# constantingoeldel/alphabeta-rs

Hardware: AMD Instinct MI355X
Metric: ABneutral model fits/sec (pedigree x bootstraps x windows) (higher is better)
Workload: dtype f64; 1 GPU; C3: synthetic 100-edge/8-generation pedigree (N=105 rows, T=8, K=47 distinct triples), 10 starts + 10000 bootstraps per GPU (bootstraps of one window sharded over the GPUs); rows=105, windows_per_gpu=1, starts=10, bootstraps=10000, plan_device_bytes=11405122, reduction_tree=0x10040, parallelism=bootstraps sharded over 1 GPU(s), one RCCL all-gather of the bootstrap tables

## Files before the change

### alphabeta_rs_amd/__init__.py

```python
from __future__ import annotations

import ctypes as C
import os
from pathlib import Path

import numpy as np

from . import build as _build

PKG = Path(__file__).resolve().parent
LIB_PATH = PKG / "libabneutral_hip.so"
if os.environ.get("ABNEUTRAL_HIP_LIB"):
    LIB_PATH = Path(os.environ["ABNEUTRAL_HIP_LIB"])

ABN_OK = 0
STATUS_NAMES = {
    0: "ABN_OK",
    1: "ABN_ERR_INVALID_ARG",
    2: "ABN_ERR_BAD_PEDIGREE",
    3: "ABN_ERR_NO_DEVICE",
    4: "ABN_ERR_HIP",
    5: "ABN_ERR_NO_FINITE_FIT",
    6: "ABN_ERR_STATE",
}
FIT_CONVERGED, FIT_MAX_ITERS, FIT_NONFINITE, FIT_TARGET = 0, 1, 2, 3
KERNEL_NAMES = {0: "none", 1: "speculative", 2: "resident", 3: "persistent", 4: "stream", 5: "two_pass",
                6: "stream_sweep"}

FIT_INFO_DTYPE = np.dtype(
    [("best_cost", "<f8"), ("iters", "<i4"), ("evals", "<i4"), ("status", "<i4"), ("lanes", "<i4")]
)

EXPORTED_SYMBOLS = [
    "abn_default_options", "abn_device_count", "abn_init", "abn_shutdown", "abn_device_info", "abn_last_error",
    "abn_status_string", "abn_version", "abn_cost_batch", "abn_fit_batch", "abn_gen_start_simplices",
    "abn_gen_boot_simplices", "abn_gen_boot_indices", "abn_ab_neutral_run", "abn_boot_model_run",
    "abn_analyze", "abn_select_best", "abn_bootstrap_rows", "abn_pairwise_divergence", "abn_plan_create", "abn_plan_destroy", "abn_plan_set_windows", "abn_plan_run",
    "abn_plan_run_phase", "abn_plan_sync", "abn_plan_tail_handed", "abn_plan_set_early_bootstraps", "abn_plan_early_bootstraps", "abn_plan_kernel_ms", "abn_plan_raw_device_ptr",
    "abn_plan_bind_raw", "abn_plan_download", "abn_plan_counters", "abn_plan_device_bytes",
    "abn_plan_set_window_ids", "abn_plan_failed_windows",
    "abn_multi_create", "abn_multi_destroy", "abn_multi_last_error", "abn_multi_set_windows", "abn_multi_run",
    "abn_multi_sync", "abn_multi_shard", "abn_multi_raw_device_ptr", "abn_multi_download", "abn_multi_counters",
    "abn_multi_rccl_available", "abn_reduction_tree", "abn_pairwise_divergence_dev", "abn_multi_set_window_ids",
    "abn_pairwise_divergence_windows", "abn_pairwise_divergence_windows_dev",
    "abn_multi_plan_shard", "abn_plan_last_kernels", "abn_multi_kernel_ms",
    "abn_packed_row_stride", "abn_pack_codes", "abn_unpack_codes", "abn_pairwise_divergence_packed",
    "abn_pairwise_divergence_packed_dev",
    "abn_pairwise_divergence_windows_packed", "abn_pairwise_divergence_windows_packed_dev",
    "abn_analyze_batch", "abn_analyze_batch_dev", "abn_plan_analyze", "abn_multi_analyze",
    "abn_windows_create", "abn_windows_destroy", "abn_windows_info", "abn_windows_stats", "abn_windows_layout",
    "abn_windows_packed", "abn_windows_packed_device_ptr", "abn_windows_pairwise",
    "abn_sites_parse", "abn_sites_destroy", "abn_sites_info", "abn_sites_fetch", "abn_sites_deferred",
    "abn_genes_create", "abn_genes_destroy", "abn_genes_choose", "abn_genes_choose_dev", "abn_windows_create_sites",
# ... 234 lines not shown
    L.abn_genes_create.argtypes = [vp, C.c_int32, i32p, i32p, i64p, u32p, u32p, u8p, C.POINTER(vp)]
    L.abn_genes_destroy.argtypes = [vp]
    L.abn_genes_choose.argtypes = [vp, C.POINTER(GeneRule), C.c_int32, i64p, i32p, u32p, u32p, u8p, u32p, u32p, u8p, dp]
    L.abn_genes_choose_dev.argtypes = [vp, C.POINTER(GeneRule), C.c_int32, i64p, vp, vp, vp, vp, vp, vp, vp, dp]
    L.abn_windows_create_sites.argtypes = [vp, C.POINTER(WindowsParams), vp, C.POINTER(GeneRule), C.c_int32, i64p, i32p,
                                           u32p, u32p, u8p, u8p, dp, C.POINTER(vp)]
    L.abn_plan_create.argtypes = [vp, op, dp, C.c_int32, C.c_int32, C.c_int32, C.c_int32, C.c_uint32, C.c_uint32,
                                  C.POINTER(vp)]
    L.abn_plan_destroy.argtypes = [vp]
    L.abn_plan_set_windows.argtypes = [vp, dp, dp, dp, dp]
    L.abn_plan_run.argtypes = [vp]
    L.abn_plan_run_phase.argtypes = [vp, C.c_int32]
    L.abn_plan_sync.argtypes = [vp]
    L.abn_plan_tail_handed.argtypes = [vp, C.POINTER(C.c_int64)]
    L.abn_plan_set_early_bootstraps.argtypes = [vp, C.c_int32]
    L.abn_plan_set_stream_sweep.argtypes = [vp, C.c_int32]
    L.abn_plan_stream_sweep.argtypes = [vp, C.POINTER(C.c_int64)]
    L.abn_multi_set_stream_sweep.argtypes = [vp, C.c_int32]
    L.abn_plan_early_bootstraps.argtypes = [vp, C.POINTER(C.c_int32)]
    L.abn_plan_kernel_ms.argtypes = [vp, dp]
    L.abn_plan_raw_device_ptr.argtypes = [vp, C.POINTER(vp)]
    L.abn_plan_bind_raw.argtypes = [vp, vp]
    L.abn_plan_download.argtypes = [vp, dp, dp, dp, dp, vp, vp, C.POINTER(C.c_int32)]
    L.abn_plan_counters.argtypes = [vp, C.POINTER(C.c_int64)]
    L.abn_plan_device_bytes.argtypes = [vp, C.POINTER(C.c_int64)]
    L.abn_plan_set_window_ids.argtypes = [vp, u32p]
    L.abn_plan_failed_windows.argtypes = [vp, C.POINTER(C.c_int32)]
    L.abn_plan_last_kernels.argtypes = [vp, C.POINTER(C.c_int32)]
    i32p = C.POINTER(C.c_int32)
    L.abn_multi_create.argtypes = [i32p, C.c_int32, op, dp, C.c_int32, C.c_int32, C.c_int32, C.c_int32, C.POINTER(vp)]
# ... 573 lines not shown

    def run_phase(self, phase: int):
        self.ctx._check(self._L.abn_plan_run_phase(self._h, phase))

    def sync(self):
        self.ctx._check(self._L.abn_plan_sync(self._h))

    def tail_handed(self):
        out = (C.c_int64 * 2)()
        self.ctx._check(self._L.abn_plan_tail_handed(self._h, out))
        return int(out[0]), int(out[1])

    def set_early_bootstraps(self, mode: int):
        self.ctx._check(self._L.abn_plan_set_early_bootstraps(self._h, mode))

    def early_bootstraps(self):
        out = (C.c_int32 * 4)()
        self.ctx._check(self._L.abn_plan_early_bootstraps(self._h, out))
        return {"eligible": bool(out[0]), "quorum": int(out[1]), "parked": int(out[2]), "miss": bool(out[3])}

    def set_stream_sweep(self, mode: int):
        self.ctx._check(self._L.abn_plan_set_stream_sweep(self._h, mode))

    def stream_sweep(self):
        out = (C.c_int64 * 4)()
        self.ctx._check(self._L.abn_plan_stream_sweep(self._h, out))
        return {"mode": int(out[0]), "starts": bool(out[1]), "boot": bool(out[2]), "passes": int(out[3])}

    def kernel_ms(self):
        ms = np.zeros(3)
# ... 684 lines not shown
```

### alphabeta_rs_amd/build.py

```python
from __future__ import annotations

import os
import shutil
import subprocess
from pathlib import Path

PKG = Path(__file__).resolve().parent
CSRC = PKG / "csrc"
LIB = PKG / "libabneutral_hip.so"
SOURCES = [CSRC / "abn_api.hip", CSRC / "abn_context.hip", CSRC / "abn_plan.hip",
           CSRC / "abn_pairwise.hip", CSRC / "abn_windows.hip", CSRC / "abn_analyze.hip",
           CSRC / "abn_multi.hip", CSRC / "abn_sites.hip", CSRC / "abn_genes.hip", CSRC / "abn_codes.hip",
           CSRC / "abn_sites_common.hip", CSRC / "abn_sites_union.hip", CSRC / "abn_tiles.hip", CSRC / "abn_blocks.hip",
           CSRC / "abn_sites_sort.hip",
           CSRC / "abn_resident.hip",
           CSRC / "abn_pack.cpp"]
DEPS = [*sorted(CSRC.glob("*.hpp")), CSRC / "abn_philox.h", PKG.parent / "include" / "abneutral.h"]
HIPCC_FLAGS = [
    "--offload-arch=gfx950",
    "-O3",
    "-std=c++17",
    "-ffp-contract=off",
    "-fno-fast-math",
    "-fPIC",
# ... 44 lines not shown
HOST = PKG / "host"
CLI = PKG / "bin" / "alphabeta"
META_CLI = PKG / "bin" / "metaprofile_alphabeta"
REF_TESTS = PKG / "bin" / "reference_tests"
PEDIGREE_LIB = PKG / "libabneutral_host.so"


def build_host(force: bool = False, verbose: bool = False) -> Path:
    build_hip()
    srcs = [HOST / "alphabeta_cli.cpp", HOST / "alphabeta.hpp", HOST / "pedigree_build.hpp", HOST / "windows_extract.hpp",
            HOST / "resident.hpp", HOST / "host_capi.cpp", HOST / "block_bootstrap.hpp",
            HOST / "metaprofile.hpp", HOST / "metaprofile_cli.cpp", HOST / "reference_tests.cpp",
            CSRC / "abn_route.hpp", CSRC / "abn_constants.hpp", CSRC / "abn_parse.hpp", CSRC / "abn_genes.hpp",
            CSRC / "abn_sites_merge.hpp", CSRC / "abn_sites_split.hpp", CSRC / "abn_sites_sort.hpp", CSRC / "abn_codes.hpp", CSRC / "abn_sites_common.hpp",
            CSRC / "abn_sites_union.hpp", CSRC / "abn_tiles.hpp", HOST / "tiles.hpp",
            CSRC / "abn_pairwise_transitions.hpp", CSRC / "abn_packed_mask.hpp", HOST / "transitions.hpp"]
    newest = max(p.stat().st_mtime for p in srcs)
    CLI.parent.mkdir(exist_ok=True)
    common = ["-O2", "-std=c++17", "-ffp-contract=off", "-Wall", "-I", str(PKG.parent / "include")]
    if force or not CLI.exists() or CLI.stat().st_mtime < newest:
        cmd = [hipcc_path(), *common, "-o", str(CLI), str(HOST / "alphabeta_cli.cpp"), "-L", str(PKG),
               "-labneutral_hip", "-Wl,-rpath,$ORIGIN/.."]
        if verbose:
            print(" ".join(cmd))
        subprocess.run(cmd, check=True, cwd=str(PKG))
    if force or not META_CLI.exists() or META_CLI.stat().st_mtime < newest:
        cmd = [hipcc_path(), *common, "-o", str(META_CLI), str(HOST / "metaprofile_cli.cpp"), "-L", str(PKG),
               "-labneutral_hip", "-Wl,-rpath,$ORIGIN/.."]
        if verbose:
            print(" ".join(cmd))
        subprocess.run(cmd, check=True, cwd=str(PKG))
# ... 19 lines not shown
```

### alphabeta_rs_amd/csrc/abn_api.hip

```cpp
#include <functional>

#include "abn_fit_host.hpp"
#include "abn_device.hpp"

using namespace abn;

static_assert(sizeof(abn_fit_info) == sizeof(FitInfoDev), "abn_fit_info layout");

static hipError_t allow_lds(const void* kernel, size_t lds) {
  if (lds <= kDefaultDynLds) return hipSuccess;
  return hipFuncSetAttribute(kernel, hipFuncAttributeMaxDynamicSharedMemorySize, (int)lds);
}

struct KernelEntry {
  KernelKey key;
  const void* fn;
};
#define ABN_FIT(G, R, TP, ST) {{kFamFit, G, R, TP, ST, false}, reinterpret_cast<const void*>(&abn_fit_kernel<G, R, TP, ST>)}
#define ABN_FIT_ROWS(G, TP, ST) ABN_FIT(G, 1, TP, ST), ABN_FIT(G, 2, TP, ST), ABN_FIT(G, 4, TP, ST), ABN_FIT(G, 8, TP, ST), ABN_FIT(G, 0, TP, ST)
#define ABN_FIT_G(G)                                                                                                   \
  ABN_FIT_ROWS(G, false, false), ABN_FIT(G, -1, false, false), ABN_FIT_ROWS(G, true, false), ABN_FIT(G, -1, true, false), \
      ABN_FIT_ROWS(G, false, true)
#define ABN_REFILL(G, R) {{kFamRefill, G, R, false, false, false}, reinterpret_cast<const void*>(&abn_fit_refill_kernel<G, R>)}
#define ABN_REFILL_G(G) ABN_REFILL(G, 1), ABN_REFILL(G, 2), ABN_REFILL(G, 4), ABN_REFILL(G, 8)
// ... 97 lines not shown
    const bool status = persistent && a.slice_status, fifo = a.quantum > 0;
    if ((status || fifo) && !lc) return set_err(c, ABN_ERR_INVALID_ARG, "internal: a persistent launch without its clears");
    if (lc) {
      bool& status_clean = lc->clean->status[lc->slot];
      bool& fifo_clean = lc->clean->fifo[lc->region];
      const PrepList l = prep_launch(lc->slot, status && !status_clean, fifo && !fifo_clean, (unsigned)a.park_cap, lc->region);
      if (int rc = clear_ranges(c, l, lc->bases, st)) return rc;
      if (status) status_clean = false;
      if (fifo) fifo_clean = false;
    }
  }
  if (int rc = launch_route(c, r, a, st)) return rc;
  if (a.tail_cap > 0) return launch_tail_resume(c, pr, a, a.tail_cap, st);
  return ABN_OK;
}

int abn::launch_select(abn_ctx* c, const SelectArgs& s, size_t lds, hipStream_t st) {
  HIPCHK(c, allow_lds(reinterpret_cast<const void*>(&abn_select_lse_kernel), lds));
  HIPCHK(c, allow_lds(reinterpret_cast<const void*>(&abn_select_kernel), lds));
  hipLaunchKernelGGL(abn_select_lse_kernel, dim3((unsigned)((long long)s.W * s.S)), dim3(kWave), lds, st, s);
  hipLaunchKernelGGL(abn_select_kernel, dim3((unsigned)s.W), dim3(kWave), lds, st, s);
  HIPCHK(c, hipGetLastError());
  return ABN_OK;
}

int abn::launch_gen_idx(abn_ctx* c, uint32_t* idx, int n, int b, int w, uint64_t seed, uint32_t woff, uint32_t boff,
                        const uint32_t* wid) {
  const long long total = (long long)w * b * ((n + 3) / 4);
  if (total <= 0) return ABN_OK;
  const long long want = (total + 255) / 256;
// ... 245 lines not shown
```

### alphabeta_rs_amd/csrc/abn_common.hpp

```cpp
#pragma once
#include <type_traits>
#include <hip/hip_runtime.h>
#include <stdint.h>

#include "abn_constants.hpp"
#include "abn_philox.h"

namespace abn {

#ifndef ABN_STREAM_WAVES
#define ABN_STREAM_WAVES 2
#endif
constexpr int kStreamWaves = ABN_STREAM_WAVES;

typedef uint32_t u32x4 __attribute__((ext_vector_type(4), aligned(4)));
typedef uint16_t u16x4 __attribute__((ext_vector_type(4), aligned(2)));
typedef double f64x2 __attribute__((ext_vector_type(2), aligned(8)));
typedef uint32_t u32x4_lds __attribute__((ext_vector_type(4)));
typedef double f64x2_lds __attribute__((ext_vector_type(2)));

constexpr int ST_INIT0 = 0;
constexpr int ST_REFLECT = 5;
constexpr int ST_EXPAND = 6;
constexpr int ST_CONTRACT = 7;
// ... 43 lines not shown
  int no_skip;
  unsigned long long* skipped;
  unsigned* queue;
  int quantum;
  unsigned park_cap;
  unsigned* park_ht;
  int* parked;
  unsigned* slice_status;
  int tail_cap;
  int spec_resume;
  unsigned* quorum_words;
  int quorum;
  const unsigned* guard;
  int guard_stop;
  int guard_poll;
#ifdef ABN_MEASUREMENT_KNOBS
  int prio_mode;
  int prio_t[3];
  int drop_entry;
#endif
  double sd_tol;
  double gap_tol;
  double* best;
  FitInfoDev* info;
  double* raw;
  unsigned long long* dbg;
  unsigned long long* passes;
};

struct SelectArgs {
// ... 264 lines not shown
__device__ __forceinline__ double cond_div(double a0, double a1, double a2, double b0, double b1, double b2) {
  return 0.5 * (a0 * b1 + a1 * b0 + a1 * b2 + a2 * b1) + (a0 * b2 + a2 * b0);
}

__device__ __forceinline__ void load_matrix(const double* m, double (&M)[9]) {
  const f64x2_lds* v = reinterpret_cast<const f64x2_lds*>(m);
#pragma unroll
  for (int e = 0; e < 4; ++e) {
    const f64x2_lds x = v[e];
    M[2 * e] = x[0];
    M[2 * e + 1] = x[1];
  }
  M[8] = m[8];
}

__device__ __forceinline__ double triple_dt(uint32_t tr, const double* pw, int TP, double sv0, double sv1,
                                            double sv2) {
  (void)TP;
  const int t0 = tr & 0xff, ea = (tr >> 8) & 0xff, eb = (tr >> 16) & 0xff;
  double P[9], A[9], B[9];
  load_matrix(pw + t0 * kPw, P);
  const double s0 = fma3(sv2, P[6], fma3(sv1, P[3], fma3(sv0, P[0], 0.0)));
  const double s1 = fma3(sv2, P[7], fma3(sv1, P[4], fma3(sv0, P[1], 0.0)));
  const double s2 = fma3(sv2, P[8], fma3(sv1, P[5], fma3(sv0, P[2], 0.0)));
  __builtin_amdgcn_sched_barrier(0);
  load_matrix(pw + ea * kPw, A);
  load_matrix(pw + eb * kPw, B);
  const double d_mm = cond_div(A[6], A[7], A[8], B[6], B[7], B[8]);
  const double d_um = cond_div(A[3], A[4], A[5], B[3], B[4], B[5]);
  const double d_uu = cond_div(A[0], A[1], A[2], B[0], B[1], B[2]);
  return s0 * d_uu + s1 * d_um + s2 * d_mm;
}

template <int I>
__device__ __forceinline__ void insert_tail(double (&c)[5], double (&v)[5]) {
  const double fi = c[I], xi = v[I];
  bool b[I];
  b[I - 1] = fi < c[I - 1];
#pragma unroll
  for (int j = I - 2; j >= 0; --j) b[j] = b[j + 1] && (fi < c[j]);
// ... 123 lines not shown
```

### alphabeta_rs_amd/csrc/abn_fit_refill.hpp

```cpp
#pragma once
#include "abn_common.hpp"
#include "abn_fit_kernel.hpp"

namespace abn {

constexpr int ST_IDLE = 13;

#ifndef ABN_REFILL_MIN_WAVES
#define ABN_REFILL_MIN_WAVES 3
#endif
typedef const __attribute__((address_space(4))) FitArgs ColdArgs;
template <int G, int RMAX>
__global__ __launch_bounds__(kWave, ABN_REFILL_MIN_WAVES) void abn_fit_refill_kernel(const FitArgs a) {
  static_assert(RMAX > 0, "resident mode only");
  constexpr int NG = kWave / G;
  constexpr int RR = RMAX;
  extern __shared__ __align__(16) double lds[];

  auto cold = [&]() {
    ColdArgs* p = (ColdArgs*)__builtin_amdgcn_kernarg_segment_ptr();
    asm volatile("" : "+s"(p));
    return p;
  };
  auto cold_v = [](int v) {
// ... 25 lines not shown
  double* dtab = pw + kPw * TP;
  double* wconst = dtab + ((K + 1) & ~1);
  double* dobs = wconst + 4;
  uint32_t* tri_s = reinterpret_cast<uint32_t*>(dobs + ((N + 1) & ~1));

  const bool canon = a.tree == kTreeCanon;
  uint32_t tidp[(RR + 1) / 2];
  for (int t = gl; t < K; t += G) tri_s[t] = a.tri[t];
#pragma unroll
  for (int q = 0; q < (RR + 1) / 2; ++q) tidp[q] = 0u;
#pragma unroll
  for (int q = 0; q < RR; ++q) {
    const int i = gl + G * q;
    if (i < N) tidp[q / 2] |= (uint32_t)a.tid[i] << (16 * (q & 1));
  }

  unsigned chain = blockIdx.x * NG + g;
  double vx[5], c[5];
  int st = ST_IDLE;
  int iter = 0, evals = 0;
  double xc = 0.0, x0 = 0.0, xr = 0.0, bx = __builtin_nan("");
  double fr = 0.0, best_cost = __builtin_inf();
  bool have_best = false;
  int fin_status = 2;
  int q_start = 0;
  bool fresh_done = false;
  bool wave_fd = false;
  bool tail_mode = false;
  bool tail_park = false;
  int skip_rest = 0;
  unsigned wstep = 0;
  unsigned gstep = 0;
#pragma unroll
  for (int k = 0; k < 5; ++k) {
    vx[k] = 0.0;
    c[k] = 0.0;
  }

  auto load_observations = [&](ColdArgs* ca, int w, int cgl) {
    const int wi = w * ca->wstride;
    const size_t wN = (size_t)w * (size_t)N;
    if (cgl == 0) {
      const double p_uu0 = ca->p_uu[wi];
      wconst[0] = p_uu0;
      wconst[1] = 1.0 - p_uu0;
      wconst[2] = ca->eqp[wi];
      wconst[3] = ca->eqp_w[wi] * (double)N;
    }
    const int dmode = ca->dmode;
    const uint32_t* idx_row = (dmode == 1) ? ca->idx + (size_t)chain * (size_t)N : nullptr;
    const size_t dN = (dmode == 2) ? (size_t)chain * (size_t)N : wN;
#pragma unroll
    for (int q = 0; q < RR; ++q) {
      const int i = cgl + G * q;
      if (i < N)
        dobs[i] = (dmode == 1) ? ca->pred[wN + i] + ca->resid[wN + idx_row[i]] : ca->D[dN + i];
    }
  };
  auto setup_chain = [&]() {
    ColdArgs* ca = cold();
    const int cgl = cold_v(gl), cdim = cgl & 3;
    const int w = (int)(chain / (unsigned)ca->C);
// ... 49 lines not shown
    fin_status = 2;
    fr = 0.0;
    double acc = vx[0];
    acc = acc + vx[1];
    acc = acc + vx[2];
    acc = acc + vx[3];
    x0 = acc * (1.0 / 4.0);
    xr = x0 + (x0 - vx[4]) * 1.0;
    xc = xr;
    q_start = evals;
    st = ST_REFLECT;
  };
  if (chain < total_of(cold())) setup_chain();
  __syncthreads();

  auto eval = [&](double xd) -> double {
    const double al = dpp_mov<kDppQuadBcast0>(xd), be = dpp_mov<kDppQuadBcast1>(xd);
    const double wt = dpp_mov<kDppQuadBcast2>(xd), ic = dpp_mov<kDppQuadBcast3>(xd);
    const double p_mm = wconst[1];
    const double sv0 = wconst[0], sv1 = wt * p_mm, sv2 = (1.0 - wt) * p_mm;
    const double puu = p_uu_est(al, be);
    const double dq = puu - wconst[2];
    const double pen = wconst[3] * (dq * dq);
    uint32_t tr = tri_s[gl < K ? gl : 0];
    const int T = (int)cold_s((unsigned)a.T);
    if constexpr (kMatrixFma && G == kWave) build_power_table_mx<G>(al, be, T, lds, a.chain_stride, dtab, lane);
    else build_power_table<G>(genmatrix(al, be), T, TP, pw, gl);
    __syncthreads();
#pragma unroll 1
    for (int t = gl; t < K; t += G) {
      const uint32_t trn = tri_s[t + G < K ? t + G : 0];
      dtab[t] = triple_dt(tr, pw, TP, sv0, sv1, sv2);
      tr = trn;
    }
    __syncthreads();
    double acc = 0.0;
    constexpr int RC = RR < 8 ? RR : 8;
    constexpr int NA = kWave / G;
    double av[NA];
#pragma unroll
    for (int j = 0; j < NA; ++j) av[j] = 0.0;
#pragma unroll
    for (int q0 = 0; q0 < RR; q0 += RC) {
      double dv[RC], tv[RC], x[RC];
#pragma unroll
      for (int q = 0; q < RC; ++q) {
        const int i = gl + G * (q0 + q);
        dv[q] = dobs[i < N ? i : N - 1];
// ... 67 lines not shown
    const bool done = status >= 0 || suspend;
    fin_status = (status >= 0) ? (have_best ? status : 2) : (suspend ? kFitSuspended : fin_status);
    double acc = vx[0];
    acc = acc + vx[1];
    acc = acc + vx[2];
    acc = acc + vx[3];
    x0 = acc * (1.0 / 4.0);
    xr = x0 + (x0 - vx[4]) * 1.0;
    xc = xr;
    st = done ? ST_DONE : ST_REFLECT;
  };

#ifdef ABN_MEASUREMENT_KNOBS
  int prio_cur = 0;
#endif
  while (__ballot(st != ST_IDLE) != 0ull) {
    bool start_shrink;
    do {
      asm volatile("; abn: hot step begin");
#ifdef ABN_MEASUREMENT_KNOBS
      if (a.prio_mode != 0) {
        const int e = st != ST_IDLE ? evals : 0;
        int m = 0;
#pragma unroll
        for (int j = 0; j < NG; ++j) {
          const int ej = __builtin_amdgcn_readlane(e, j * G);
          m = ej > m ? ej : m;
        }
        int lvl = (m >= a.prio_t[0] ? 1 : 0) + (m >= a.prio_t[1] ? 1 : 0) + (m >= a.prio_t[2] ? 1 : 0);
        if (a.prio_mode == 2) lvl = 3 - lvl;
        if (lvl != prio_cur) {
// ... 12 lines not shown
          const unsigned total = total_of(ca);
          const unsigned fq = __hip_atomic_load(ca->queue, __ATOMIC_RELAXED, __HIP_MEMORY_SCOPE_AGENT);
          const int av = __hip_atomic_load(reinterpret_cast<int*>(park_header(ca)) + kParkAvail, __ATOMIC_RELAXED, __HIP_MEMORY_SCOPE_AGENT);
          const unsigned fin = __hip_atomic_load(ca->slice_status + kSliceFinished, __ATOMIC_RELAXED, __HIP_MEMORY_SCOPE_AGENT);
          t = (slots() + fq >= total && av <= 0 && total - fin <= (unsigned)ca->tail_cap) ? 1 : 0;
        }
        tail_mode = __builtin_amdgcn_readfirstlane(t) != 0;
      }
      const int gmask = (int)cold_s((unsigned)guard_mask);
      const bool guard_due = gmask >= 0 && (++gstep & (unsigned)gmask) == 0u;
      int guard_stop_now = 0;
      if (guard_due) {
        if (cold_v(lane) == 0) guard_stop_now = guard_says_stop() ? 1 : 0;
      }
      const bool in_init = st < ST_REFLECT;
      const double f = eval(in_init ? vx[0] : xc);
      if (guard_due && __builtin_amdgcn_readfirstlane(guard_stop_now) != 0) return;
      const bool is_ref = st == ST_REFLECT, is_exp = st == ST_EXPAND, is_con = st == ST_CONTRACT;
      const bool active = is_ref || is_exp || is_con;
      const bool acc_r = is_ref && (f < c[3]) && (f >= c[0]);
      const bool go_exp = is_ref && !acc_r && (f < c[0]);
      const bool go_con = is_ref && !acc_r && !go_exp && (f >= c[3]);
      const bool nan_ref = is_ref && !acc_r && !go_exp && !go_con;
      const bool keep_r = is_exp && !(f < fr);
      const bool acc_c = is_con && (f < c[4]);
      const bool rej_c = is_con && !acc_c;
      const bool do_insert = acc_r || is_exp || acc_c;
      const int shrink_variant = (int)cold_s((unsigned)a.shrink_variant);
      start_shrink = nan_ref || (rej_c && shrink_variant != 0);
      const bool do_begin = do_insert || (rej_c && shrink_variant == 0);
      evals += active ? 1 : 0;
// ... 22 lines not shown
        for (int q = 0; q < 4; ++q) {
          c[q] = c[q + 1];
          vx[q] = vx[q + 1];
        }
        c[4] = f;
        vx[4] = tv;
        st = st + 1;
        if (st == ST_REFLECT) {
          evals = 5;
          sort5(c, vx);
          begin_iteration(false);
        }
      }
      asm volatile("; abn: hot step end");
    } while (__ballot(start_shrink || st == ST_DONE) == 0ull);
    if (__ballot(start_shrink) != 0ull) {
#pragma unroll 1
      for (int k = 1; k < 5; ++k) {
        const double nv = vx[0] + (vx[1] - vx[0]) * 0.5;
        const double fk = eval(start_shrink ? nv : xc);
        if (start_shrink) {
          ++evals;
#pragma unroll
          for (int q = 1; q < 4; ++q) {
            c[q] = c[q + 1];
            vx[q] = vx[q + 1];
          }
          c[4] = fk;
          vx[4] = nv;
        }
      }
      if (start_shrink) {
        sort5(c, vx);
        begin_iteration(true);
      }
// ... 123 lines not shown
```

### alphabeta_rs_amd/csrc/abn_plan.hip

```cpp
#include "abn_fit_host.hpp"
#include "abn_plan_kernels.hpp"

using namespace abn;

enum PlanEvent { kEvFitA, kEvSelect, kEvSelectEnd, kEvFitB, kEvFitBOwn, kEvFitBEnd, kPlanEvents };
struct EventSpan {
  int begin, end;
};

struct PhaseRecord {
  EventSpan span;
  bool ran = false;
  int32_t kind = 0, lanes = 0;
  long long expected = 0;
  long long handed = 0;
  bool sweep = false;
};
struct EarlyRecord {
  bool ran = false;
  int32_t parked = 0, miss = 0;
};

struct abn_plan {
  abn_ctx* ctx = nullptr;
// ... 23 lines not shown
  hipEvent_t ev[kPlanEvents] = {};
  PhaseRecord rec[2] = {{{kEvFitA, kEvSelect}}, {{kEvFitB, kEvFitBEnd}}};
  EventSpan select_span{kEvSelect, kEvSelectEnd};
  EarlyRecord early_rec;
  PrepClean clean;
  hipEvent_t ev_fork = nullptr;
  std::vector<hipEvent_t> ev_join;
  EarlyRoute early{};
  int early_mode = 1;
  DevBuf<double> early_state;
  DevBuf<int> early_list;
  DevBuf<double> sel_model, sel_pred, sel_resid;
  DevBuf<int32_t> sel_best;
  int sweep_mode = 0;
  DevBuf<unsigned long long> sweep_passes;
};

static unsigned* early_words(const abn_plan* p) { return reinterpret_cast<unsigned*>(p->skipped.p + kPhaseSlots * kPhaseWords); }
static unsigned* slice_words(const abn_plan* p, int slot) { return early_words(p) + kEarlyWords + kSliceWords * slot; }
struct PlanWordsHost {
  unsigned long long phase[kPhaseSlots][kPhaseWords];
  unsigned early[kEarlyWords];
  unsigned slice[kPhaseSlots][kSliceWords];
};
static_assert(offsetof(PlanWordsHost, early) == kPlanEarlyOffset && offsetof(PlanWordsHost, slice) == plan_status_offset(0) &&
                  offsetof(PlanWordsHost, slice[kSlotRedo]) == plan_status_offset(kSlotRedo),
              "abn_prepare.hpp addresses the same words");
static_assert(sizeof(PlanWordsHost) <= kPlanWords64 * sizeof(unsigned long long) && sizeof(PlanWordsHost) % 8 == 0 &&
                  offsetof(PlanWordsHost, early) == kPhaseSlots * kPhaseWords * sizeof(unsigned long long) &&
                  offsetof(PlanWordsHost, slice) == offsetof(PlanWordsHost, early) + kEarlyWords * sizeof(unsigned),
// ... 196 lines not shown
  a.pred = p->pred.p + o.rows;
  a.resid = p->resid.p + o.rows;
  a.idx = p->idx.p + o.boots * (size_t)p->N;
  a.model = p->model.p + o.w * 4;
  a.window_offset = p->window_offset + (uint32_t)w0;
  a.boot_offset = p->boot_offset;
  a.wid = p->wid.p ? p->wid.p + o.w : nullptr;
  a.W = wn;
  a.C = phase ? p->B : p->S;
  a.dmode = a.smode = phase;
  a.simplex0 = phase ? nullptr : p->simplexA.p + chains * 20;
  a.max_iters = phase ? p->opt.max_iters_boot : p->opt.max_iters_start;
  a.best = (phase ? p->bestB.p : p->bestA.p) + chains * 4;
  a.info = (phase ? p->infoB.p : p->infoA.p) + chains;
  a.raw = phase ? p->raw + chains * 7 : nullptr;
  return a;
}

static PrepBases prep_bases(const abn_plan* p) {
  PrepBases b;
  b.base[kPrepWords] = p->skipped.p;
  b.bytes[kPrepWords] = p->skipped.bytes();
  b.base[kPrepFifo] = p->slice_buf.p;
  b.bytes[kPrepFifo] = p->slice_buf.bytes();
  b.base[kPrepSweep] = p->sweep_passes.p;
  b.bytes[kPrepSweep] = p->sweep_passes.bytes();
  b.base[kPrepTail] = p->susp_list.p;
  b.bytes[kPrepTail] = p->susp_list.bytes();
  return b;
}
// ... 248 lines not shown
  if (int rc = enqueue_phase_b(p, 0, p->W, c->stream, false, true, g)) return rc;
  HIPCHK(c, hipEventRecord(p->ev[kEvFitBEnd], c->stream));
  end_step(p, true, true, true);
  return ABN_OK;
}

static bool early_applies(const abn_plan* p) { return p->early.eligible && p->early_mode != 0; }

extern "C" int abn_plan_set_early_bootstraps(abn_plan* p, int32_t mode) {
  if (!p) return ABN_ERR_INVALID_ARG;
  if (mode != 0 && mode != 1) return set_err(p->ctx, ABN_ERR_INVALID_ARG, "early bootstraps: mode must be 0 (off) or 1 (auto)");
  p->early_mode = mode;
  return ABN_OK;
}

static int verify_persistent(abn_plan* p);

extern "C" int abn_plan_set_stream_sweep(abn_plan* p, int32_t mode) {
  if (!p) return ABN_ERR_INVALID_ARG;
  abn_ctx* c = p->ctx;
  if (mode != 0 && mode != 1) return set_err(c, ABN_ERR_INVALID_ARG, "stream sweep: mode must be 0 (off) or 1 (on)");
  if (mode == 1 && !p->sweep_passes.p) {
    HIPCHK(c, hipSetDevice(c->device));
    PoolScope pool_scope(c);
    hipError_t e = p->sweep_passes.alloc(2);
    if (e != hipSuccess) return set_err(c, ABN_ERR_HIP, std::string("hipMalloc sweep_passes: ") + hipGetErrorString(e));
    PrepList l;
    l.add(kPrepSweep, 0, p->sweep_passes.bytes(), 0x00);
    if (int rc = clear_ranges(c, l, prep_bases(p), c->stream, false)) return rc;
  }
// ... 283 lines not shown
```

### alphabeta_rs_amd/host/host_capi.cpp

```cpp
#include <chrono>
#include <cstring>
#include <memory>

#include "../csrc/abn_genes.hpp"
#include "../csrc/abn_parse.hpp"
#include "../csrc/abn_route.hpp"
#include "../csrc/abn_codes.hpp"
#include "../csrc/abn_pairwise_transitions.hpp"
#include "../csrc/abn_sites_merge.hpp"
#include "../csrc/abn_sites_split.hpp"
#include "../csrc/abn_sites_sort.hpp"
#include "../csrc/abn_sites_common.hpp"
#include "../csrc/abn_sites_union.hpp"
#include "../csrc/abn_tiles.hpp"
#include "alphabeta.hpp"
#include "tiles.hpp"

namespace {
struct DiagCapture {
  std::string text;
  std::string* const found = alphabeta::detail::diag_sink();
  DiagCapture() { alphabeta::detail::diag_sink() = &text; }
  ~DiagCapture() { alphabeta::detail::diag_sink() = found; }
};
// ... 24 lines not shown
  } catch (const std::exception& e) {
    return failed(err, errcap, e);
  }
}
int abh_pedigree_build(const char* nodelist, const char* edgelist, double posterior_max_filter, double* rows, int cap,
                       double* p0uu, char* err, int errcap) {
  return pedigree_build(nodelist, edgelist, posterior_max_filter, false, false, nullptr, rows, cap, p0uu, err, errcap);
}
int abh_pedigree_build_gpu(const char* nodelist, const char* edgelist, double posterior_max_filter, const char* out_path,
                           double* rows, int cap, double* p0uu, char* err, int errcap) {
  return pedigree_build(nodelist, edgelist, posterior_max_filter, true, false, out_path, rows, cap, p0uu, err, errcap);
}
long long abh_packed_scan_calls() { return alphabeta::detail::packed_scan_calls().load(); }
long long abh_packed_windows_scan_calls() { return alphabeta::detail::packed_windows_scan_calls().load(); }
long long abh_resident_build_calls() { return alphabeta::detail::resident_build_calls().load(); }
int abh_pedigree_build_resident(const char* nodelist, const char* edgelist, double posterior_max_filter, const char* out_path,
                                double* rows, int cap, double* p0uu, char* err, int errcap) {
  return pedigree_build(nodelist, edgelist, posterior_max_filter, true, true, out_path, rows, cap, p0uu, err, errcap);
}
int abh_pedigree_build_ab(const char* nodelist, const char* edgelist, const char* const* texts, const long long* lens, int n,
                          double posterior_max_filter, int which, double* ms2, double* kernel_ms4, char* err, int errcap) {
  try {
    static std::vector<std::string> held;
    if (n > 0) {
      held.clear();
      for (int i = 0; i < n; ++i) held.emplace_back(texts[i], (size_t)lens[i]);
    }
    DiagCapture quiet;
    std::pair<alphabeta::Pedigree, double> host, device;
    if (which & 1) {
// ... 788 lines not shown
```

### include/abneutral.h

```cpp
#ifndef ABNEUTRAL_H
#define ABNEUTRAL_H

#include <stdint.h>

#ifdef __cplusplus
extern "C" {
#endif

#define ABN_VERSION_MAJOR 0
#define ABN_VERSION_MINOR 1

typedef enum abn_status {
  ABN_OK = 0,
  ABN_ERR_INVALID_ARG = 1,
  ABN_ERR_BAD_PEDIGREE = 2,
  ABN_ERR_NO_DEVICE = 3,
  ABN_ERR_HIP = 4,
  ABN_ERR_NO_FINITE_FIT = 5,
  ABN_ERR_STATE = 6
} abn_status;

#define ABN_FIT_CONVERGED 0
#define ABN_FIT_MAX_ITERS 1
#define ABN_FIT_NONFINITE 2
// ... 287 lines not shown
int abn_tiles_block_ms(const abn_tiles* h, double* ms5);

int abn_plan_create(abn_ctx* ctx, const abn_options* opts, const double* generations ,
                    int32_t n_rows, int32_t n_windows, int32_t n_starts, int32_t n_boot,
                    uint32_t window_offset, uint32_t boot_offset, abn_plan** plan);
int abn_plan_destroy(abn_plan* plan);
int abn_plan_set_window_ids(abn_plan* plan, const uint32_t* ids);
int abn_plan_set_windows(abn_plan* plan, const double* d_obs, const double* p0uu, const double* eqp,
                         const double* eqp_weight);
int abn_plan_run(abn_plan* plan);
int abn_plan_run_phase(abn_plan* plan, int32_t phase );
int abn_plan_sync(abn_plan* plan);
int abn_plan_tail_handed(abn_plan* plan, int64_t* out2);
int abn_plan_set_early_bootstraps(abn_plan* plan, int32_t mode);
int abn_plan_early_bootstraps(abn_plan* plan, int32_t* out4);
int abn_plan_set_stream_sweep(abn_plan* plan, int32_t mode);
int abn_plan_stream_sweep(abn_plan* plan, int64_t* out4);
int abn_plan_kernel_ms(abn_plan* plan, double* ms3);
int abn_plan_raw_device_ptr(abn_plan* plan, void** dev_ptr);
int abn_plan_bind_raw(abn_plan* plan, void* dev_ptr);
int abn_plan_download(abn_plan* plan, double* models, double* pred, double* resid, double* raw,
                      abn_fit_info* info_a, abn_fit_info* info_b, int32_t* best_start);
int abn_plan_analyze(abn_plan* plan, double* out, int32_t* first_bad);
int abn_plan_failed_windows(abn_plan* plan, int32_t* n_failed);
int abn_plan_counters(abn_plan* plan, int64_t* out5);
int abn_plan_device_bytes(abn_plan* plan, int64_t* bytes);
#define ABN_KERNEL_NONE 0
#define ABN_KERNEL_SPECULATIVE 1
#define ABN_KERNEL_RESIDENT 2
#define ABN_KERNEL_PERSISTENT 3
// ... 32 lines not shown
```

Measured before the change: 3.541 million fits/s.

## Share drain-phase triple evaluation across live chains in a wave

New measurement: 3.552 million fits/s, median of 4. Within noise of the previous version (+0.3%).

```diff
diff --git a/alphabeta_rs_amd/__init__.py b/alphabeta_rs_amd/__init__.py
--- a/alphabeta_rs_amd/__init__.py
+++ b/alphabeta_rs_amd/__init__.py
@@ -36,7 +36,7 @@
     "abn_status_string", "abn_version", "abn_cost_batch", "abn_fit_batch", "abn_gen_start_simplices",
     "abn_gen_boot_simplices", "abn_gen_boot_indices", "abn_ab_neutral_run", "abn_boot_model_run",
     "abn_analyze", "abn_select_best", "abn_bootstrap_rows", "abn_pairwise_divergence", "abn_plan_create", "abn_plan_destroy", "abn_plan_set_windows", "abn_plan_run",
-    "abn_plan_run_phase", "abn_plan_sync", "abn_plan_tail_handed", "abn_plan_set_early_bootstraps", "abn_plan_early_bootstraps", "abn_plan_kernel_ms", "abn_plan_raw_device_ptr",
+    "abn_plan_run_phase", "abn_plan_sync", "abn_plan_tail_handed", "abn_plan_set_early_bootstraps", "abn_plan_early_bootstraps", "abn_plan_set_drain_share", "abn_plan_kernel_ms", "abn_plan_raw_device_ptr",
     "abn_plan_bind_raw", "abn_plan_download", "abn_plan_counters", "abn_plan_device_bytes",
     "abn_plan_set_window_ids", "abn_plan_failed_windows",
     "abn_multi_create", "abn_multi_destroy", "abn_multi_last_error", "abn_multi_set_windows", "abn_multi_run",
@@ -301,6 +301,7 @@
     L.abn_plan_sync.argtypes = [vp]
     L.abn_plan_tail_handed.argtypes = [vp, C.POINTER(C.c_int64)]
     L.abn_plan_set_early_bootstraps.argtypes = [vp, C.c_int32]
+    L.abn_plan_set_drain_share.argtypes = [vp, C.c_int32]
     L.abn_plan_set_stream_sweep.argtypes = [vp, C.c_int32]
     L.abn_plan_stream_sweep.argtypes = [vp, C.POINTER(C.c_int64)]
     L.abn_multi_set_stream_sweep.argtypes = [vp, C.c_int32]
@@ -904,6 +905,9 @@
     def set_early_bootstraps(self, mode: int):
         self.ctx._check(self._L.abn_plan_set_early_bootstraps(self._h, mode))
 
+    def set_drain_share(self, mode: int):
+        self.ctx._check(self._L.abn_plan_set_drain_share(self._h, mode))
+
     def early_bootstraps(self):
         out = (C.c_int32 * 4)()
         self.ctx._check(self._L.abn_plan_early_bootstraps(self._h, out))
diff --git a/alphabeta_rs_amd/build.py b/alphabeta_rs_amd/build.py
--- a/alphabeta_rs_amd/build.py
+++ b/alphabeta_rs_amd/build.py
@@ -82,7 +82,8 @@
             CSRC / "abn_route.hpp", CSRC / "abn_constants.hpp", CSRC / "abn_parse.hpp", CSRC / "abn_genes.hpp",
             CSRC / "abn_sites_merge.hpp", CSRC / "abn_sites_split.hpp", CSRC / "abn_sites_sort.hpp", CSRC / "abn_codes.hpp", CSRC / "abn_sites_common.hpp",
             CSRC / "abn_sites_union.hpp", CSRC / "abn_tiles.hpp", HOST / "tiles.hpp",
-            CSRC / "abn_pairwise_transitions.hpp", CSRC / "abn_packed_mask.hpp", HOST / "transitions.hpp"]
+            CSRC / "abn_pairwise_transitions.hpp", CSRC / "abn_packed_mask.hpp", HOST / "transitions.hpp",
+            CSRC / "abn_drain_share.hpp"]
     newest = max(p.stat().st_mtime for p in srcs)
     CLI.parent.mkdir(exist_ok=True)
     common = ["-O2", "-std=c++17", "-ffp-contract=off", "-Wall", "-I", str(PKG.parent / "include")]
diff --git a/alphabeta_rs_amd/csrc/abn_api.hip b/alphabeta_rs_amd/csrc/abn_api.hip
--- a/alphabeta_rs_amd/csrc/abn_api.hip
+++ b/alphabeta_rs_amd/csrc/abn_api.hip
@@ -135,6 +135,15 @@
   if (a.tail_cap > 0) return launch_tail_resume(c, pr, a, a.tail_cap, st);
   return ABN_OK;
 }
+
+#ifdef ABN_MEASUREMENT_KNOBS
+extern "C" int abn_knobs_drain_shared_steps(unsigned long long* steps, int reset) {
+  const unsigned long long zero = 0;
+  if (steps && hipMemcpyFromSymbol(steps, HIP_SYMBOL(g_drain_shared_steps), sizeof(*steps)) != hipSuccess) return ABN_ERR_HIP;
+  if (reset && hipMemcpyToSymbol(HIP_SYMBOL(g_drain_shared_steps), &zero, sizeof(zero)) != hipSuccess) return ABN_ERR_HIP;
+  return ABN_OK;
+}
+#endif
 
 int abn::launch_select(abn_ctx* c, const SelectArgs& s, size_t lds, hipStream_t st) {
   HIPCHK(c, allow_lds(reinterpret_cast<const void*>(&abn_select_lse_kernel), lds));
diff --git a/alphabeta_rs_amd/csrc/abn_common.hpp b/alphabeta_rs_amd/csrc/abn_common.hpp
--- a/alphabeta_rs_amd/csrc/abn_common.hpp
+++ b/alphabeta_rs_amd/csrc/abn_common.hpp
@@ -81,6 +81,7 @@
   const unsigned* guard;
   int guard_stop;
   int guard_poll;
+  int drain_share;
 #ifdef ABN_MEASUREMENT_KNOBS
   int prio_mode;
   int prio_t[3];
@@ -375,6 +376,7 @@
   M[8] = m[8];
 }
 
+template <bool LEAN = false>
 __device__ __forceinline__ double triple_dt(uint32_t tr, const double* pw, int TP, double sv0, double sv1,
                                             double sv2) {
   (void)TP;
@@ -385,6 +387,25 @@
   const double s1 = fma3(sv2, P[7], fma3(sv1, P[4], fma3(sv0, P[1], 0.0)));
   const double s2 = fma3(sv2, P[8], fma3(sv1, P[5], fma3(sv0, P[2], 0.0)));
   __builtin_amdgcn_sched_barrier(0);
+  if constexpr (LEAN) {
+    const f64x2_lds* va = reinterpret_cast<const f64x2_lds*>(pw + ea * kPw);
+    const f64x2_lds* vb = reinterpret_cast<const f64x2_lds*>(pw + eb * kPw);
+#pragma unroll
+    for (int e = 0; e < 3; ++e) {
+      const f64x2_lds x = va[e], y = vb[e];
+      A[2 * e] = x[0];
+      A[2 * e + 1] = x[1];
+      B[2 * e] = y[0];
+      B[2 * e + 1] = y[1];
+    }
+    const double d_um = cond_div(A[3], A[4], A[5], B[3], B[4], B[5]);
+    const double d_uu = cond_div(A[0], A[1], A[2], B[0], B[1], B[2]);
+    const double head = s0 * d_uu + s1 * d_um;
+    __builtin_amdgcn_sched_barrier(0);
+    const f64x2_lds x = va[3], y = vb[3];
+    const double d_mm = cond_div(x[0], x[1], pw[ea * kPw + 8], y[0], y[1], pw[eb * kPw + 8]);
+    return head + s2 * d_mm;
+  }
   load_matrix(pw + ea * kPw, A);
   load_matrix(pw + eb * kPw, B);
   const double d_mm = cond_div(A[6], A[7], A[8], B[6], B[7], B[8]);
diff --git a/alphabeta_rs_amd/csrc/abn_drain_share.hpp b/alphabeta_rs_amd/csrc/abn_drain_share.hpp
--- /dev/null
+++ b/alphabeta_rs_amd/csrc/abn_drain_share.hpp
@@ -0,0 +1,54 @@
+#pragma once
+#include "abn_constants.hpp"
+
+namespace abn {
+
+constexpr int kDrainShare = 1;
+constexpr int kDrainSlots = 8;
+
+constexpr unsigned drain_group_mask(unsigned long long lanes, int G) {
+  unsigned m = 0;
+  for (int j = 0; j < kWave / G; ++j) m |= (unsigned)((lanes >> (j * G)) & 1ull) << j;
+  return m;
+}
+constexpr int drain_live(unsigned gmask) {
+  int n = 0;
+  for (int j = 0; j < kDrainSlots; ++j) n += (gmask >> j) & 1u;
+  return n;
+}
+constexpr unsigned drain_pack(unsigned gmask) {
+  unsigned p = 0, first = 0;
+  int n = 0;
+  for (int j = kDrainSlots - 1; j >= 0; --j)
+    if ((gmask >> j) & 1u) first = (unsigned)j;
+  for (int j = 0; j < kDrainSlots; ++j)
+    if ((gmask >> j) & 1u) p |= (unsigned)j << (3 * n++);
+  for (; n < kDrainSlots; ++n) p |= first << (3 * n);
+  return p;
+}
+constexpr int drain_rounds(int L, int K) { return (L * K + kWave - 1) / kWave; }
+constexpr int drain_items(int G, int K, int L) { return (L > 0 && drain_rounds(L, K) < (K + G - 1) / G) ? L * K : 0; }
+
+struct DrainAt {
+  int slot, tri;
+};
+constexpr DrainAt drain_first(int lane, int K) { return {lane / K, lane % K}; }
+constexpr DrainAt drain_next(DrainAt at, int q64, int r64, int K) {
+  const int t = at.tri + r64;
+  return t >= K ? DrainAt{at.slot + q64 + 1, t - K} : DrainAt{at.slot + q64, t};
+}
+constexpr int drain_group(unsigned pack, int slot) { return (int)((pack >> (3 * (slot < kDrainSlots ? slot : kDrainSlots - 1))) & 7u); }
+constexpr unsigned drain_word(int G, int K, unsigned gmask) {
+  const int L = drain_live(gmask);
+  return drain_items(G, K, L) != 0 ? (unsigned)L << 24 | drain_pack(gmask) : 0u;
+}
+
+constexpr int drain_serve(int G, int K, unsigned gmask, int lane, int round) {
+  const int items = drain_items(G, K, drain_live(gmask));
+  DrainAt at = drain_first(lane, K);
+  for (int r = 0; r < round; ++r) at = drain_next(at, kWave / K, kWave % K, K);
+  if (lane + kWave * round >= items) return -1;
+  return drain_group(drain_pack(gmask), at.slot) << 16 | at.tri;
+}
+
+}
diff --git a/alphabeta_rs_amd/csrc/abn_fit_refill.hpp b/alphabeta_rs_amd/csrc/abn_fit_refill.hpp
--- a/alphabeta_rs_amd/csrc/abn_fit_refill.hpp
+++ b/alphabeta_rs_amd/csrc/abn_fit_refill.hpp
@@ -1,10 +1,14 @@
 #pragma once
 #include "abn_common.hpp"
 #include "abn_fit_kernel.hpp"
+#include "abn_drain_share.hpp"
 
 namespace abn {
 
 constexpr int ST_IDLE = 13;
+#ifdef ABN_MEASUREMENT_KNOBS
+static __device__ unsigned long long g_drain_shared_steps;
+#endif
 
 #ifndef ABN_REFILL_MIN_WAVES
 #define ABN_REFILL_MIN_WAVES 3
@@ -63,6 +67,9 @@
     const int i = gl + G * q;
     if (i < N) tidp[q / 2] |= (uint32_t)a.tid[i] << (16 * (q & 1));
   }
+
+  const int drain_at0 = cold_v((int)((unsigned)(lane / K) << 16 | (unsigned)(lane % K)));
+  const int drain_step = cold_v((int)((unsigned)a.chain_stride << 14 | (unsigned)(kWave / K) << 7 | (unsigned)(kWave % K)));
 
   unsigned chain = blockIdx.x * NG + g;
   double vx[5], c[5];
@@ -80,6 +87,9 @@
   int skip_rest = 0;
   unsigned wstep = 0;
   unsigned gstep = 0;
+#ifdef ABN_MEASUREMENT_KNOBS
+  unsigned shared_steps = 0;
+#endif
 #pragma unroll
   for (int k = 0; k < 5; ++k) {
     vx[k] = 0.0;
@@ -94,7 +104,7 @@
       wconst[0] = p_uu0;
       wconst[1] = 1.0 - p_uu0;
       wconst[2] = ca->eqp[wi];
-      wconst[3] = ca->eqp_w[wi] * (double)N;
+      wconst[3] = ca->eqp_w[wi] * (double)ca->N;
     }
     const int dmode = ca->dmode;
     const uint32_t* idx_row = (dmode == 1) ? ca->idx + (size_t)chain * (size_t)N : nullptr;
@@ -174,7 +184,7 @@
   if (chain < total_of(cold())) setup_chain();
   __syncthreads();
 
-  auto eval = [&](double xd) -> double {
+  auto eval = [&](double xd, unsigned share) -> double {
     const double al = dpp_mov<kDppQuadBcast0>(xd), be = dpp_mov<kDppQuadBcast1>(xd);
     const double wt = dpp_mov<kDppQuadBcast2>(xd), ic = dpp_mov<kDppQuadBcast3>(xd);
     const double p_mm = wconst[1];
@@ -187,11 +197,33 @@
     if constexpr (kMatrixFma && G == kWave) build_power_table_mx<G>(al, be, T, lds, a.chain_stride, dtab, lane);
     else build_power_table<G>(genmatrix(al, be), T, TP, pw, gl);
     __syncthreads();
+    if (share != 0u) {
+      const int step = (int)cold_s((unsigned)__builtin_amdgcn_readfirstlane(drain_step)), at0 = cold_v(drain_at0);
+      const unsigned pack = cold_s(share);
+      const int stride = step >> 14, q64 = (step >> 7) & 127, r64 = step & 127;
+      const unsigned items = (pack >> 24) * (unsigned)K;
+      DrainAt at{at0 >> 16, at0 & 0xffff};
+#ifdef ABN_MEASUREMENT_KNOBS
+      ++shared_steps;
+#endif
 #pragma unroll 1
-    for (int t = gl; t < K; t += G) {
-      const uint32_t trn = tri_s[t + G < K ? t + G : 0];
-      dtab[t] = triple_dt(tr, pw, TP, sv0, sv1, sv2);
-      tr = trn;
+      for (unsigned base = 0; base < items; base += kWave) {
+        const int sg = drain_group(pack, at.slot);
+        const int d = (sg - g) * stride;
+        const double* wcs = wconst + d;
+        const double wts = lane_fetch(xd, sg * G + 2);
+        const double pmm = wcs[1];
+        const double dt = triple_dt<true>(tri_s[at.tri], pw + d, TP, wcs[0], wts * pmm, (1.0 - wts) * pmm);
+        if (base + (unsigned)lane < items) dtab[d + at.tri] = dt;
+        at = drain_next(at, q64, r64, K);
+      }
+    } else {
+#pragma unroll 1
+      for (int t = gl; t < K; t += G) {
+        const uint32_t trn = tri_s[t + G < K ? t + G : 0];
+        dtab[t] = triple_dt(tr, pw, TP, sv0, sv1, sv2);
+        tr = trn;
+      }
     }
     __syncthreads();
     double acc = 0.0;
@@ -289,7 +321,9 @@
 #ifdef ABN_MEASUREMENT_KNOBS
   int prio_cur = 0;
 #endif
-  while (__ballot(st != ST_IDLE) != 0ull) {
+  unsigned long long live_lanes;
+  while ((live_lanes = __ballot(st != ST_IDLE)) != 0ull) {
+    const unsigned share = cold()->drain_share != 0 ? drain_word(G, K, drain_group_mask(live_lanes, G)) : 0u;
     bool start_shrink;
     do {
       asm volatile("; abn: hot step begin");
@@ -332,7 +366,7 @@
         if (cold_v(lane) == 0) guard_stop_now = guard_says_stop() ? 1 : 0;
       }
       const bool in_init = st < ST_REFLECT;
-      const double f = eval(in_init ? vx[0] : xc);
+      const double f = eval(in_init ? vx[0] : xc, share);
       if (guard_due && __builtin_amdgcn_readfirstlane(guard_stop_now) != 0) return;
       const bool is_ref = st == ST_REFLECT, is_exp = st == ST_EXPAND, is_con = st == ST_CONTRACT;
       const bool active = is_ref || is_exp || is_con;
@@ -385,11 +419,15 @@
       }
       asm volatile("; abn: hot step end");
     } while (__ballot(start_shrink || st == ST_DONE) == 0ull);
+#ifdef ABN_MEASUREMENT_KNOBS
+    if (shared_steps != 0u && cold_v(lane) == 0) atomicAdd(&g_drain_shared_steps, (unsigned long long)shared_steps);
+    shared_steps = 0u;
+#endif
     if (__ballot(start_shrink) != 0ull) {
 #pragma unroll 1
       for (int k = 1; k < 5; ++k) {
         const double nv = vx[0] + (vx[1] - vx[0]) * 0.5;
-        const double fk = eval(start_shrink ? nv : xc);
+        const double fk = eval(start_shrink ? nv : xc, 0u);
         if (start_shrink) {
           ++evals;
 #pragma unroll
diff --git a/alphabeta_rs_amd/csrc/abn_plan.hip b/alphabeta_rs_amd/csrc/abn_plan.hip
--- a/alphabeta_rs_amd/csrc/abn_plan.hip
+++ b/alphabeta_rs_amd/csrc/abn_plan.hip
@@ -1,4 +1,5 @@
 #include "abn_fit_host.hpp"
+#include "abn_drain_share.hpp"
 #include "abn_plan_kernels.hpp"
 
 using namespace abn;
@@ -61,6 +62,7 @@
   DevBuf<int32_t> sel_best;
   int sweep_mode = 0;
   DevBuf<unsigned long long> sweep_passes;
+  int drain_share = kDrainShare;
 };
 
 static unsigned* early_words(const abn_plan* p) { return reinterpret_cast<unsigned*>(p->skipped.p + kPhaseSlots * kPhaseWords); }
@@ -287,6 +289,7 @@
   a.best = (phase ? p->bestB.p : p->bestA.p) + chains * 4;
   a.info = (phase ? p->infoB.p : p->infoA.p) + chains;
   a.raw = phase ? p->raw + chains * 7 : nullptr;
+  a.drain_share = p->drain_share;
   return a;
 }
 
@@ -565,6 +568,13 @@
   return ABN_OK;
 }
 
+extern "C" int abn_plan_set_drain_share(abn_plan* p, int32_t mode) {
+  if (!p) return ABN_ERR_INVALID_ARG;
+  if (mode != 0 && mode != 1) return set_err(p->ctx, ABN_ERR_INVALID_ARG, "drain sharing: mode must be 0 (off) or 1 (on)");
+  p->drain_share = mode;
+  return ABN_OK;
+}
+
 static int verify_persistent(abn_plan* p);
 
 extern "C" int abn_plan_set_stream_sweep(abn_plan* p, int32_t mode) {
diff --git a/alphabeta_rs_amd/host/host_capi.cpp b/alphabeta_rs_amd/host/host_capi.cpp
--- a/alphabeta_rs_amd/host/host_capi.cpp
+++ b/alphabeta_rs_amd/host/host_capi.cpp
@@ -6,6 +6,7 @@
 #include "../csrc/abn_parse.hpp"
 #include "../csrc/abn_route.hpp"
 #include "../csrc/abn_codes.hpp"
+#include "../csrc/abn_drain_share.hpp"
 #include "../csrc/abn_pairwise_transitions.hpp"
 #include "../csrc/abn_sites_merge.hpp"
 #include "../csrc/abn_sites_split.hpp"
@@ -62,6 +63,15 @@
 long long abh_packed_scan_calls() { return alphabeta::detail::packed_scan_calls().load(); }
 long long abh_packed_windows_scan_calls() { return alphabeta::detail::packed_windows_scan_calls().load(); }
 long long abh_resident_build_calls() { return alphabeta::detail::resident_build_calls().load(); }
+int abh_drain_serve(int lanes_per_chain, int k, unsigned live_groups, int lane, int round) {
+  return abn::drain_serve(lanes_per_chain, k, live_groups, lane, round);
+}
+int abh_drain_rounds(int live, int k) { return abn::drain_rounds(live, k); }
+int abh_drain_items(int lanes_per_chain, int k, int live) { return abn::drain_items(lanes_per_chain, k, live); }
+void abh_drain_table(int lanes_per_chain, int k, unsigned live_groups, int rounds, int* out) {
+  for (int r = 0; r < rounds; ++r)
+    for (int l = 0; l < abn::kWave; ++l) out[r * abn::kWave + l] = abn::drain_serve(lanes_per_chain, k, live_groups, l, r);
+}
 int abh_pedigree_build_resident(const char* nodelist, const char* edgelist, double posterior_max_filter, const char* out_path,
                                 double* rows, int cap, double* p0uu, char* err, int errcap) {
   return pedigree_build(nodelist, edgelist, posterior_max_filter, true, true, out_path, rows, cap, p0uu, err, errcap);
diff --git a/include/abneutral.h b/include/abneutral.h
--- a/include/abneutral.h
+++ b/include/abneutral.h
@@ -325,6 +325,7 @@
 int abn_plan_tail_handed(abn_plan* plan, int64_t* out2);
 int abn_plan_set_early_bootstraps(abn_plan* plan, int32_t mode);
 int abn_plan_early_bootstraps(abn_plan* plan, int32_t* out4);
+int abn_plan_set_drain_share(abn_plan* plan, int32_t mode);
 int abn_plan_set_stream_sweep(abn_plan* plan, int32_t mode);
 int abn_plan_stream_sweep(abn_plan* plan, int64_t* out4);
 int abn_plan_kernel_ms(abn_plan* plan, double* ms3);
```
